# kaiwenShen/Do-You-Really-Need-to-Pay-2-20-Hedge-Fund-Strategy-Replication-via-Machine-Learning

Hardware: AMD Instinct MI355X
Metric: seq/sec/node MTSS-WGAN-GP train (24x32 windows) at 1/2/4/8 GPUs; W-dist parity (higher is better)
Workload: dtype fp32; 1 GPU; global_batch=262144, batch_per_gpu=262144, seq_len=24, features=32, parallelism=dp1

## Files before the change

do-you-really-need-to-pay-2-20-hedge-fund-strategy-replication-via-machine-learning_amd/csrc/lstm_f32.hip:

```cpp
#include "lstmf_dev.h"

#include <atomic>
#include <cstdlib>
#include <type_traits>
#include <stdexcept>

namespace hfrep {

namespace {

__device__ __forceinline__ rsrc_t ftile_rsrc(const float* base, int row0, int B, int Tn, int W) {
  row0 = __builtin_amdgcn_readfirstlane(row0);
  const int nr = base ? max(0, min(32, B - row0)) : 0;
  return make_rsrc(base + (nr ? (size_t)row0 * Tn * W : 0), nr * Tn * W * 4);
}

template <int K>
struct FGeo {
  static_assert(K >= 1 && K <= 112, "fp32 LSTM: K <= 112");
  static constexpr int KS = (K + 3) / 4;
  static constexpr int KQ = KS <= 12 ? 12 : 28;
  static constexpr int LR = KS <= 12 ? 56 : 120;
  static constexpr int NJ = (KS + 3) / 4;
};
// ... 965 lines not shown
            if (!tok) { cdn = 0.f; hd = 0.f; }
            cst[m][n] = cdn;
            cprev[m][n] = c;
            hv = hd;
            st4(f32x4{zd[0], zd[1], zd[2], zd[3]}, rt, tok ? tl + tb + ftape_slot(m, n) : kOOB);
            st1(cdn, rt, tok ? tcl + tb + ftape_slot(m, n) : kOOB, 0);
          }
          {
            const int u = ub + 4 * n, row = 16 * m + 4 * g + q;
            const uint32_t h1 = trunc_hi(hv);
            const float r1 = hv - __builtin_bit_cast(float, h1);
            const uint32_t m1 = trunc_hi(r1);
            const uint32_t l1 = __builtin_bit_cast(uint32_t, r1 - __builtin_bit_cast(float, m1));
            const bool pl = u < 96;
            lds_char* dp = pl ? hnext + (row * FS_HR + u) * 2 : trashc;
            *reinterpret_cast<__attribute__((address_space(3))) uint16_t*>(dp) = (uint16_t)(h1 >> 16);
            *reinterpret_cast<__attribute__((address_space(3))) uint16_t*>(dp + (pl ? FS_HPL : 0)) = (uint16_t)(m1 >> 16);
            *reinterpret_cast<__attribute__((address_space(3))) uint16_t*>(dp + (pl ? 2 * FS_HPL : 0)) = (uint16_t)(l1 >> 16);
            const bool tl4 = u >= 96 && u < FH;
            lds_char* tp = tl4 ? hnext + 3 * FS_HPL + (row * 4 + (u - 96)) * 4 : trashc;
            *reinterpret_cast<__attribute__((address_space(3))) float*>(tp) = hv;
          }
          st1(hv, rh, v1, 0);
        }
      }
      xp.to_lds(xb + ((t + 1) & 1) * 32 * GX::LR, trash);
      lds_barrier();
    }
  }
}

#ifndef HFREP_FWDS2_SKEW
#define HFREP_FWDS2_SKEW 0
#endif
constexpr int F2_TILES = 25;
__device__ __forceinline__ float f2_rnd(float v) {
  asm("" : "+v"(v));
  return v;
}
template <int KX>
constexpr size_t fwds2_smem() {
  return (size_t)(2 * 32 * FGeo<KX>::LR + 4) * 4 + 2 * FS_HB + (size_t)F2_TILES * FGeo<KX>::NJ * 64 * 16;
}

template <int ACT, int KX, bool TAPE, bool TAN, int NT, bool HI, bool FLIP>
__device__ __forceinline__ void fwds2_run(const float* __restrict__ x, const float* __restrict__ W,
                                          const float* __restrict__ bias, const float* __restrict__ U,
                                          const float* __restrict__ ptape, float* __restrict__ hs,
                                          float* __restrict__ tape, int B, int Tn, float* fsm, int v) {
  using GX = FGeo<KX>;
  float* xb = fsm;
  float* trash = xb + 2 * 32 * GX::LR;
  lds_char* hb = (lds_char*)(trash + 4);
  f32x4* wl = (f32x4*)(hb + 2 * FS_HB);
  const int tid = threadIdx.x, lane = tid & 63;
  const int q = lane & 3, g = lane >> 4, j4 = (lane & 15) >> 2;
  const int t0 = v ? 3 * v + 1 : 0;
  const int ub = 4 * t0 + j4;
  const int nrb = (B + 31) / 32;
  const int flip = (FLIP && v >= 4) ? 1 : 0;

  for (int i = tid; i < 2 * 32 * GX::LR; i += 512) xb[i] = 0.f;

  constexpr float GSC = ACT == ACT_TANH ? -2.f * kLog2e : ACT == ACT_SIGMOID ? -kLog2e : 1.f;
  const float sc = TAN ? 1.f : (q == 2 ? GSC : -kLog2e);
  bf16x8 up[3][NT][3];
  float ut[NT], bq[NT];
  int tsl[NT];
#pragma unroll
  for (int n = 0; n < NT; ++n) {
    const int cl = q * FH + ub + 4 * n;
    tsl[n] = ftape_lane((t0 + n) / FNT, 0) + (((t0 + n) % FNT) * FT_SLOT) * 4;
#pragma unroll
    for (int ks = 0; ks < 3; ++ks) {
      uint32_t hh[8], mm[8], ll[8];
#pragma unroll
      for (int j = 0; j < 8; ++j) {
        const int k = 32 * ks + 8 * g + j;
        const float u_ = f2_rnd(U[k * FG + cl] * sc);
        const uint32_t h = trunc_hi(u_);
        const float r1 = u_ - __builtin_bit_cast(float, h);
        const uint32_t m = trunc_hi(r1);
        const float r2 = r1 - __builtin_bit_cast(float, m);
        hh[j] = h; mm[j] = m; ll[j] = __builtin_bit_cast(uint32_t, r2);
      }
      uint4 ph, pm, pl;
      ph.x = __builtin_amdgcn_perm(hh[1], hh[0], 0x07060302u); ph.y = __builtin_amdgcn_perm(hh[3], hh[2], 0x07060302u);
      ph.z = __builtin_amdgcn_perm(hh[5], hh[4], 0x07060302u); ph.w = __builtin_amdgcn_perm(hh[7], hh[6], 0x07060302u);
      pm.x = __builtin_amdgcn_perm(mm[1], mm[0], 0x07060302u); pm.y = __builtin_amdgcn_perm(mm[3], mm[2], 0x07060302u);
      pm.z = __builtin_amdgcn_perm(mm[5], mm[4], 0x07060302u); pm.w = __builtin_amdgcn_perm(mm[7], mm[6], 0x07060302u);
      pl.x = __builtin_amdgcn_perm(ll[1], ll[0], 0x07060302u); pl.y = __builtin_amdgcn_perm(ll[3], ll[2], 0x07060302u);
      pl.z = __builtin_amdgcn_perm(ll[5], ll[4], 0x07060302u); pl.w = __builtin_amdgcn_perm(ll[7], ll[6], 0x07060302u);
      up[ks][n][0] = __builtin_bit_cast(bf16x8, ph);
      up[ks][n][1] = __builtin_bit_cast(bf16x8, pm);
      up[ks][n][2] = __builtin_bit_cast(bf16x8, pl);
#pragma unroll
      for (int p = 0; p < 3; ++p) asm volatile("" : "+v"(up[ks][n][p]));
    }
    ut[n] = U[(96 + g) * FG + cl] * sc;
#pragma unroll
    for (int j = 0; j < GX::NJ; ++j) {
      f32x4 wv;
#pragma unroll
      for (int s4 = 0; s4 < 4; ++s4) {
        const int k = 4 * (4 * j + s4) + g;
        const float w_ = W[min(k, KX - 1) * FG + cl];
        wv[s4] = k < KX ? w_ * sc : 0.f;
      }
      wl[((t0 + n) * GX::NJ + j) * 64 + lane] = wv;
    }
    const float bv = bias ? bias[cl] : 0.f;
    bq[n] = !TAN ? f2_rnd(bv * sc) : 0.f;
  }
  const bool glin = !TAN && ACT == ACT_LINEAR && q == 2;
  const float am = (ACT == ACT_TANH && q == 2) ? 2.f : 1.f, bm = (ACT == ACT_TANH && q == 2) ? -1.f : 0.f;
  const int ax = (lane & 15) * GX::LR + g * GX::KQ;
  const int ahp = ((lane & 15) * FS_HR + 8 * g) * 2, aht = 3 * FS_HPL + ((lane & 15) * 4 + g) * 4;
  const f32x4* wlw = wl + t0 * GX::NJ * 64 + lane;
  FXPart<KX> xp;
  const bool xld = v >= 4;

  for (int rb = blockIdx.x; rb < nrb; rb += gridDim.x) {
    const int row0 = rb * 32;
    const rsrc_t rx = ftile_rsrc(x, row0, B, Tn, KX);
    const rsrc_t rh = ftile_rsrc(hs, row0, B, Tn, FH);
    const rsrc_t rt = ftape_rsrc(TAPE ? tape : nullptr, rb, nrb, Tn);
    const rsrc_t rp = ftape_rsrc(TAN ? ptape : nullptr, rb, nrb, Tn);
    const int vp0 = ((4 * g + q) * Tn * FH + ub) * 4;
    float cprev[TAN ? 2 : 1][NT];
    if constexpr (TAN) {
#pragma unroll
      for (int i = 0; i < 2; ++i)
#pragma unroll
        for (int n = 0; n < NT; ++n) cprev[i][n] = 0.f;
    }
    float cst[2][NT];
#pragma unroll
    for (int i = 0; i < 2; ++i)
#pragma unroll
      for (int n = 0; n < NT; ++n) cst[i][n] = 0.f;
    xp.set(Tn, tid & 255);
    if (!xld) {
#pragma unroll
      for (int j = 0; j < FXPart<KX>::NJ; ++j) { xp.goff[j] = kOOB; xp.lpos[j] = -1; }
    }
    xp.load(rx, Tn, 0, true);
    for (int i = tid; i < FS_HB / 16; i += 512)
      reinterpret_cast<__attribute__((address_space(3))) u32x4_t*>(hb)[i] = u32x4_t{0, 0, 0, 0};
    xp.to_lds(xb, trash);
    __syncthreads();
    for (int t = 0; t < Tn; ++t) {
      const float* xcur = xb + (t & 1) * 32 * GX::LR;
      const lds_char* hcur = hb + (t & 1) * FS_HB;
      lds_char* hnext = hb + ((t + 1) & 1) * FS_HB;
      xp.load(rx, Tn, t + 1, t + 1 < Tn);
#pragma unroll
      for (int i = 0; i < 2; ++i) {
        const int m = i ^ flip;
        f32x4 pg[TAN ? NT : 1];
        float pc[TAN ? NT : 1];
        const int p1 = vp0 + (16 * m * Tn + t) * FH * 4;
        const int tb = t * FT_STEP * 4 + m * ftape_slot(1, 0);
        if constexpr (TAN) {
#pragma unroll
          for (int n = 0; n < NT; ++n) {
            pg[n] = ld4(rp, lane * 16 + (tb + tsl[n]));
            pc[n] = ld1(rp, (256 + lane) * 4 + (tb + tsl[n]), 0);
          }
        }
        f32x4 acc[NT];
#pragma unroll
        for (int n = 0; n < NT; ++n) acc[n] = f32x4{0.f, 0.f, 0.f, 0.f};
        if constexpr (HI) __builtin_amdgcn_s_setprio(1);
#pragma unroll
        for (int j = 0; j < GX::NJ; ++j) {
          const f32x4 a4 = *reinterpret_cast<const f32x4*>(xcur + ax + 16 * m * GX::LR + 4 * j);
          f32x4 w4[NT];
#pragma unroll
          for (int n = 0; n < NT; ++n) w4[n] = wlw[(n * GX::NJ + j) * 64];
#pragma unroll
          for (int s4 = 0; s4 < 4; ++s4) {
            const int ks = 4 * j + s4;
            if (ks >= GX::KS) break;
#pragma unroll
            for (int n = 0; n < NT; ++n) acc[n] = mma4(a4[s4], w4[n][s4], acc[n]);
          }
          __builtin_amdgcn_sched_barrier(0);
        }
#pragma unroll
        for (int ks = 0; ks < 3; ++ks) {
          const lds_char* ar = hcur + ahp + 16 * m * FS_HR * 2 + 64 * ks;
          const bf16x8 a[3] = {*reinterpret_cast<const __attribute__((address_space(3))) bf16x8*>(ar),
                               *reinterpret_cast<const __attribute__((address_space(3))) bf16x8*>(ar + FS_HPL),
                               *reinterpret_cast<const __attribute__((address_space(3))) bf16x8*>(ar + 2 * FS_HPL)};
#pragma unroll
          for (int n = 0; n < NT; ++n) acc[n] = mma_split6(a, up[ks][n], acc[n]);
          __builtin_amdgcn_sched_barrier(0);
        }
        {
          const float at = *reinterpret_cast<const __attribute__((address_space(3))) float*>(hcur + aht + 16 * m * 16);
#pragma unroll
          for (int n = 0; n < NT; ++n) acc[n] = mma4(at, ut[n], acc[n]);
        }
        if constexpr (HI) __builtin_amdgcn_s_setprio(0);
#pragma unroll
        for (int n = 0; n < NT; ++n) {
          const int v1 = p1 + 16 * n;
          const int tg = lane * 16 + (tb + tsl[n]), tc = (256 + lane) * 4 + (tb + tsl[n]);
          const bool fa = (t0 + n) % FNT < 4;
          const f32x4 zs = acc[n];
          float hv, hr;
          if constexpr (!TAN) {
            float y[4];
#pragma unroll
            for (int e4 = 0; e4 < 4; ++e4) {
              const float s_ = zs[e4] + bq[n];
              const float e = __builtin_fmaf(am, __builtin_amdgcn_rcpf(1.f + __builtin_amdgcn_exp2f(s_)), bm);
              y[e4] = glin ? s_ : e;
            }
            quad_transpose(y, q);
            const float cn = __builtin_fmaf(y[1], cst[i][n], y[0] * y[2]);
            float ca;
            if constexpr (ACT == ACT_TANH) ca = __builtin_fmaf(__builtin_amdgcn_rcpf(1.f + __builtin_amdgcn_exp2f(GSC * cn)), 2.f, -1.f);
            else if constexpr (ACT == ACT_SIGMOID) ca = __builtin_amdgcn_rcpf(1.f + __builtin_amdgcn_exp2f(GSC * cn));
            else ca = cn;
            hv = f2_rnd(y[3] * ca);
            const float hh = __builtin_bit_cast(float, trunc_hi(hv));
            hr = fa ? __builtin_fmaf(y[3], ca, -hh) : hv - hh;
            cst[i][n] = cn;
            if constexpr (TAPE) {
              st4(f32x4{y[0], y[1], y[2], y[3]}, rt, tg);
              st1(cn, rt, tc, 0);
            }
          } else {
            float zd[4] = {zs[0], zs[1], zs[2], zs[3]};
            quad_transpose(zd, q);
            const f32x4 y = pg[n];
            const float idot = y[0] * (1.f - y[0]) * zd[0], fdot = y[1] * (1.f - y[1]) * zd[1];
            const float dg = ACT == ACT_TANH ? __builtin_fmaf(-y[2], y[2], 1.f) : ACT == ACT_SIGMOID ? y[2] * (1.f - y[2]) : 1.f;
            const float gdot = dg * zd[2], odot = y[3] * (1.f - y[3]) * zd[3];
            const float c = pc[n];
            const float ca = act_f(ACT, c);
            const float dc = ACT == ACT_TANH ? __builtin_fmaf(-ca, ca, 1.f) : ACT == ACT_SIGMOID ? ca * (1.f - ca) : 1.f;
            const float yd = y[3] * dc;
            float cdn, hd;
            if (fa) {
              if constexpr (ACT == ACT_LINEAR) {
                cdn = f2_rnd(y[0] * gdot) + __builtin_fmaf(idot, y[2], __builtin_fmaf(fdot, cprev[i][n], y[1] * cst[i][n]));
              } else {
                cdn = __builtin_fmaf(y[0], gdot, f2_rnd(idot * y[2]) + (f2_rnd(y[1] * cst[i][n]) + f2_rnd(fdot * cprev[i][n])));
              }
              hd = f2_rnd(odot * ca) + f2_rnd(yd * cdn);
            } else {
              cdn = __builtin_fmaf(y[0], gdot, __builtin_fmaf(idot, y[2], __builtin_fmaf(y[1], cst[i][n], fdot * cprev[i][n])));
              hd = __builtin_fmaf(odot, ca, yd * cdn);
            }
            cst[i][n] = cdn;
            cprev[i][n] = c;
            hv = hd;
            hr = hv - __builtin_bit_cast(float, trunc_hi(hv));
            st4(f32x4{zd[0], zd[1], zd[2], zd[3]}, rt, tg);
            st1(cdn, rt, tc, 0);
          }
          {
            const int row = 16 * m + 4 * g + q;
            if (t0 + n < 24) {
              const uint32_t h1 = trunc_hi(hv);
              const uint32_t m1 = trunc_hi(hr);
              const uint32_t l1 = __builtin_bit_cast(uint32_t, hr - __builtin_bit_cast(float, m1));
              lds_char* dp = hnext + (row * FS_HR + ub + 4 * n) * 2;
              *reinterpret_cast<__attribute__((address_space(3))) uint16_t*>(dp) = (uint16_t)(h1 >> 16);
              *reinterpret_cast<__attribute__((address_space(3))) uint16_t*>(dp + FS_HPL) = (uint16_t)(m1 >> 16);
              *reinterpret_cast<__attribute__((address_space(3))) uint16_t*>(dp + 2 * FS_HPL) = (uint16_t)(l1 >> 16);
            } else {
              *reinterpret_cast<__attribute__((address_space(3))) float*>(hnext + 3 * FS_HPL + (row * 4 + j4) * 4) = hv;
            }
          }
          st1(hv, rh, v1, 0);
        }
      }
      xp.to_lds(xb + ((t + 1) & 1) * 32 * GX::LR, trash);
      lds_barrier();
    }
  }
}

template <int ACT, int KX, bool TAPE, bool TAN, int SKEW>
__global__ void __launch_bounds__(512, 1)
lstmf_fwds2_kernel(const float* __restrict__ x, const float* __restrict__ W, const float* __restrict__ bias,
                   const float* __restrict__ U, const float* __restrict__ ptape, float* __restrict__ hs,
                   float* __restrict__ tape, int B, int Tn) {
  static_assert(FGeo<KX>::KS <= 12, "split forward: K <= 48");
  extern __shared__ __attribute__((aligned(16))) float fsm[];
  constexpr bool PRIO = SKEW & 1, FLIP = SKEW & 2;
  const int v = __builtin_amdgcn_readfirstlane(threadIdx.x >> 6);
  if (v == 0) fwds2_run<ACT, KX, TAPE, TAN, 4, false, FLIP>(x, W, bias, U, ptape, hs, tape, B, Tn, fsm, v);
  else if (!PRIO || v < 4) fwds2_run<ACT, KX, TAPE, TAN, 3, false, FLIP>(x, W, bias, U, ptape, hs, tape, B, Tn, fsm, v);
  else fwds2_run<ACT, KX, TAPE, TAN, 3, true, FLIP>(x, W, bias, U, ptape, hs, tape, B, Tn, fsm, v);
}

constexpr int F2_NWR3 = 13, F2_NWR4 = 5;
constexpr int F2_G3 = (25 - F2_NWR3) / 4, F2_G4 = (25 - F2_NWR4) / 4;
static_assert(F2_NWR3 + 4 * F2_G3 == 25 && F2_NWR4 + 4 * F2_G4 == 25, "W^T k-steps in LDS come in fours");
__device__ __forceinline__ constexpr int f2_woff(int gt) { return gt < 4 ? F2_G4 * gt : F2_G3 * gt + (F2_G4 - F2_G3) * 4; }
constexpr size_t fwd2_smem() {
  return (size_t)(2 * 32 * (FGeo<100>::LR + FGeo<FH>::LR) + 4) * 4 + (size_t)(F2_G3 * 25 + (F2_G4 - F2_G3) * 4) * 1024;
}

template <int ACT, bool TAPE, bool TAN, int NT>
__device__ __forceinline__ void fwd2_run(const float* __restrict__ x, const float* __restrict__ W,
                                         const float* __restrict__ bias, const float* __restrict__ U,
                                         const float* __restrict__ ptape, float* __restrict__ hs,
                                         float* __restrict__ tape, int B, int Tn, float* fsm, int v) {
  constexpr int KX = 100;
  using GX = FGeo<KX>;
  using GH = FGeo<FH>;
  constexpr bool BIG = NT == 4;
  constexpr int NWR = BIG ? F2_NWR4 : F2_NWR3, NG = BIG ? F2_G4 : F2_G3;
  static_assert(GX::KS == 25 && GH::KS == 25 && (NT == 3 || NT == 4), "tile plan of the K = 100 layer");
  float* xb = fsm;
  float* hb = xb + 2 * 32 * GX::LR;
  float* trash = hb + 2 * 32 * GH::LR;
  f32x4* wl = (f32x4*)(trash + 4);
  const int tid = threadIdx.x, lane = tid & 63;
  const int q = lane & 3, g = lane >> 4, j4 = (lane & 15) >> 2;
  const int t0 = v ? 3 * v + 1 : 0;
  const int nrb = (B + 31) / 32;

  for (int i = tid; i < 2 * 32 * (GX::LR + GH::LR); i += 512) fsm[i] = 0.f;

  constexpr float GSC = ACT == ACT_TANH ? -2.f * kLog2e : ACT == ACT_SIGMOID ? -kLog2e : 1.f;
  const float sc = TAN ? 1.f : (q == 2 ? GSC : -kLog2e);
  float uf[GH::KS][NT], wf[NWR][NT], bq[NT];
  int tsl[NT];
#pragma unroll
  for (int n = 0; n < NT; ++n) {
    const int gt = t0 + n;
    const int cl = q * FH + 4 * gt + j4;
    tsl[n] = ftape_lane(gt / FNT, 0) + ((gt % FNT) * FT_SLOT) * 4;
#pragma unroll
    for (int ks = 0; ks < GH::KS; ++ks) {
      uf[ks][n] = U[(4 * ks + g) * FG + cl] * sc;
      asm volatile("" : "+v"(uf[ks][n]));
    }
#pragma unroll
    for (int ks = 0; ks < NWR; ++ks) {
      wf[ks][n] = W[(4 * ks + g) * FG + cl] * sc;
      asm volatile("" : "+v"(wf[ks][n]));
    }
#pragma unroll
    for (int gi = 0; gi < NG; ++gi) {
      f32x4 wv;
#pragma unroll
      for (int s4 = 0; s4 < 4; ++s4) wv[s4] = W[(4 * (NWR + 4 * gi + s4) + g) * FG + cl] * sc;
      wl[(f2_woff(gt) + gi) * 64 + lane] = wv;
    }
    const float bv = bias ? bias[cl] : 0.f;
    bq[n] = !TAN ? f2_rnd(bv * sc) : 0.f;
  }
  const bool glin = !TAN && ACT == ACT_LINEAR && q == 2;
  const float am = q == 2 ? 2.f : 1.f, bm = q == 2 ? -1.f : 0.f;
  const int ax = (lane & 15) * GX::LR + g * GX::KQ, ah = (lane & 15) * GH::LR + g * GH::KQ;
  const int hw = (4 * g + q) * GH::LR + j4 * GH::KQ + t0;
  const f32x4* wlw = wl + f2_woff(t0) * 64 + lane;
  FXPart<KX> xp;
  const bool xld = v >= 4;
  __syncthreads();

  for (int rb = blockIdx.x; rb < nrb; rb += gridDim.x) {
    const int row0 = rb * 32;
    const rsrc_t rx = ftile_rsrc(x, row0, B, Tn, KX);
    const rsrc_t rh = ftile_rsrc(hs, row0, B, Tn, FH);
    const rsrc_t rt = ftape_rsrc(TAPE ? tape : nullptr, rb, nrb, Tn);
    const rsrc_t rp = ftape_rsrc(TAN ? ptape : nullptr, rb, nrb, Tn);
    const int vp0 = ((4 * g + q) * Tn * FH + 4 * t0 + j4) * 4;
    float cprev[TAN ? 2 : 1][NT];
    if constexpr (TAN) {
#pragma unroll
      for (int m = 0; m < 2; ++m)
#pragma unroll
        for (int n = 0; n < NT; ++n) cprev[m][n] = 0.f;
    }
    float cst[2][NT];
#pragma unroll
    for (int m = 0; m < 2; ++m)
#pragma unroll
      for (int n = 0; n < NT; ++n) cst[m][n] = 0.f;
    if constexpr (!BIG) {
      xp.set(Tn, tid & 255);
      if (!xld) {
#pragma unroll
        for (int j = 0; j < FXPart<KX>::NJ; ++j) { xp.goff[j] = kOOB; xp.lpos[j] = -1; }
      }
      xp.load(rx, Tn, 0, true);
    }
    for (int i = tid; i < 32 * GH::LR; i += 512) hb[i] = 0.f;
    if constexpr (!BIG) xp.to_lds(xb, trash);
    __syncthreads();
    for (int t = 0; t < Tn; ++t) {
      const float* xcur = xb + (t & 1) * 32 * GX::LR;
      const float* hcur = hb + (t & 1) * 32 * GH::LR;
      float* hnext = hb + ((t + 1) & 1) * 32 * GH::LR;
      if constexpr (!BIG) xp.load(rx, Tn, t + 1, t + 1 < Tn);
#pragma unroll
      for (int m = 0; m < 2; ++m) {
        f32x4 pg[TAN ? NT : 1];
        float pc[TAN ? NT : 1];
        const int p1 = vp0 + (16 * m * Tn + t) * FH * 4;
        const int tb = t * FT_STEP * 4 + ftape_slot(m, 0);
        if constexpr (TAN) {
#pragma unroll
          for (int n = 0; n < NT; ++n) {
            pg[n] = ld4(rp, lane * 16 + (tb + tsl[n]));
            pc[n] = ld1(rp, (256 + lane) * 4 + (tb + tsl[n]), 0);
          }
        }
        f32x4 acc[NT];
#pragma unroll
        for (int n = 0; n < NT; ++n) acc[n] = f32x4{0.f, 0.f, 0.f, 0.f};
        f32x4 w4[NT];
#pragma unroll
        for (int j = 0; j < GX::NJ; ++j) {
          const f32x4 a4 = *reinterpret_cast<const f32x4*>(xcur + ax + 16 * m * GX::LR + 4 * j);
#pragma unroll
          for (int s = 0; s < 4; ++s) {
            const int ks = 4 * j + s;
            if (ks >= GX::KS) break;
            if (ks >= NWR && (ks - NWR) % 4 == 0) {
#pragma unroll
              for (int n = 0; n < NT; ++n) w4[n] = wlw[(n * NG + (ks - NWR) / 4) * 64];
            }
#pragma unroll
            for (int n = 0; n < NT; ++n) {
              const float bw = ks < NWR ? wf[ks < NWR ? ks : 0][n] : w4[n][(ks >= NWR ? ks - NWR : 0) & 3];
              acc[n] = mma4(a4[s], bw, acc[n]);
            }
          }
          __builtin_amdgcn_sched_barrier(0);
        }
#pragma unroll
        for (int j = 0; j < GH::NJ; ++j) {
          const f32x4 a4 = *reinterpret_cast<const f32x4*>(hcur + ah + 16 * m * GH::LR + 4 * j);
#pragma unroll
          for (int s = 0; s < 4; ++s) {
            const int ks = 4 * j + s;
            if (ks >= GH::KS) break;
#pragma unroll
            for (int n = 0; n < NT; ++n) acc[n] = mma4(a4[s], uf[ks][n], acc[n]);
          }
          __builtin_amdgcn_sched_barrier(0);
        }
#pragma unroll
        for (int n = 0; n < NT; ++n) {
          const int v1 = p1 + 16 * n;
          const int tg = lane * 16 + (tb + tsl[n]), tc = (256 + lane) * 4 + (tb + tsl[n]);
          const f32x4 zs = acc[n];
          float hv;
          if constexpr (!TAN) {
            float y[4];
#pragma unroll
            for (int e4 = 0; e4 < 4; ++e4) {
              const float s_ = zs[e4] + bq[n];
              const float r_ = __builtin_amdgcn_rcpf(1.f + __builtin_amdgcn_exp2f(s_));
              float e = r_;
              if constexpr (ACT == ACT_TANH) e = __builtin_fmaf(am, r_, bm);
              y[e4] = glin ? s_ : e;
            }
            quad_transpose(y, q);
            const float cn = __builtin_fmaf(y[1], cst[m][n], y[0] * y[2]);
            float ca;
            if constexpr (ACT == ACT_TANH) ca = __builtin_fmaf(__builtin_amdgcn_rcpf(1.f + __builtin_amdgcn_exp2f(GSC * cn)), 2.f, -1.f);
            else if constexpr (ACT == ACT_SIGMOID) ca = __builtin_amdgcn_rcpf(1.f + __builtin_amdgcn_exp2f(GSC * cn));
            else ca = cn;
            hv = y[3] * ca;
            cst[m][n] = cn;
            if constexpr (TAPE) {
              st4(f32x4{y[0], y[1], y[2], y[3]}, rt, tg);
              st1(cn, rt, tc, 0);
            }
          } else {
            float zd[4] = {zs[0], zs[1], zs[2], zs[3]};
            quad_transpose(zd, q);
            const f32x4 y = pg[n];
            const float idot = y[0] * (1.f - y[0]) * zd[0], fdot = y[1] * (1.f - y[1]) * zd[1];
            const float dg = ACT == ACT_TANH ? __builtin_fmaf(-y[2], y[2], 1.f) : ACT == ACT_SIGMOID ? y[2] * (1.f - y[2]) : 1.f;
            const float gdot = dg * zd[2], odot = y[3] * (1.f - y[3]) * zd[3];
            const float c = pc[n];
            const float ca = act_f(ACT, c);
            const float dc = ACT == ACT_TANH ? __builtin_fmaf(-ca, ca, 1.f) : ACT == ACT_SIGMOID ? ca * (1.f - ca) : 1.f;
            const float yd = y[3] * dc;
            const float fc = __builtin_fmaf(fdot, cprev[m][n], y[1] * cst[m][n]);
            float cdn = __builtin_fmaf(y[0], gdot, __builtin_fmaf(idot, y[2], fc));
            if (m == 0 && (t0 + n) % FNT == 4) {
              if constexpr (ACT == ACT_LINEAR) cdn = f2_rnd(y[0] * gdot) + (f2_rnd(idot * y[2]) + (f2_rnd(fdot * cprev[m][n]) + f2_rnd(y[1] * cst[m][n])));
              else cdn = __builtin_fmaf(y[0], gdot, f2_rnd(idot * y[2]) + fc);
            }
            hv = __builtin_fmaf(odot, ca, yd * cdn);
            cst[m][n] = cdn;
            cprev[m][n] = c;
            st4(f32x4{zd[0], zd[1], zd[2], zd[3]}, rt, tg);
            st1(cdn, rt, tc, 0);
          }
          hnext[hw + 16 * m * GH::LR + n] = hv;
          st1(hv, rh, v1, 0);
        }
      }
      if constexpr (!BIG) xp.to_lds(xb + ((t + 1) & 1) * 32 * GX::LR, trash);
      lds_barrier();
    }
  }
}

template <int ACT, int KX, bool TAPE, bool TAN>
__global__ void __launch_bounds__(512, 1)
lstmf_fwd2_kernel(const float* __restrict__ x, const float* __restrict__ W, const float* __restrict__ bias,
                  const float* __restrict__ U, const float* __restrict__ ptape, float* __restrict__ hs,
                  float* __restrict__ tape, int B, int Tn) {
  static_assert(KX == 100, "the eight-wave exact forward is the K = 100 layer's");
  extern __shared__ __attribute__((aligned(16))) float fsm[];
  const int v = __builtin_amdgcn_readfirstlane(threadIdx.x >> 6);
  if (v == 0) fwd2_run<ACT, TAPE, TAN, 4>(x, W, bias, U, ptape, hs, tape, B, Tn, fsm, v);
  else fwd2_run<ACT, TAPE, TAN, 3>(x, W, bias, U, ptape, hs, tape, B, Tn, fsm, v);
}

constexpr int BS_LZ = 432;
constexpr int BS_PL = 32 * BS_LZ * 2;

template <int ACT, bool HEAD = false, bool AHD = false>
__global__ void __launch_bounds__(256, 1)
lstmf_bwds_kernel(const float* __restrict__ dH, const float* __restrict__ tape, const float* __restrict__ U,
                  float* __restrict__ dZ, int B, int Tn, const float* __restrict__ hd, const float* __restrict__ hw,
                  float* __restrict__ aH) {
  extern __shared__ __attribute__((aligned(16))) float fsm[];
  float* zt = fsm;
  float* ht = zt + 32 * BZ_LR;
  float* trash = ht + 32 * BH_LR;
  lds_char* trashp = (lds_char*)(trash + 4 * BZ_KQ);
  lds_char* zp = (lds_char*)(trash + 4 * BZ_KQ + 4);
  const int tid = threadIdx.x, lane = tid & 63;
  const int w = __builtin_amdgcn_readfirstlane(tid >> 6);
  const int q = lane & 3, g = lane >> 4, j4 = (lane & 15) >> 2, c16 = lane & 15;
  const int nrb = (B + 31) / 32;
  bf16x8 up[2][DS_KS][3];
#pragma unroll
  for (int e = 0; e < 2; ++e) {
    const int col = 16 * (2 * w + e) + c16;
    const bool ok = col < FH;
#pragma unroll
    for (int ks = 0; ks < DS_KS; ++ks) {
      f32x4 v[2];
#pragma unroll
      for (int j = 0; j < 8; ++j) {
        const int k = min(32 * ks + 8 * g + j, FG - 1);
        const float x = U[(ok ? col : 0) * FG + (k & 3) * FH + (k >> 2)];
        v[j >> 2][j & 3] = (ok && 32 * ks + 8 * g + j < FG) ? x : 0.f;
      }
      uint32_t p0[3][2], p1[3][2];
      split3(v[0], p0);
      split3(v[1], p1);
#pragma unroll
      for (int p = 0; p < 3; ++p) {
        up[e][ks][p] = __builtin_bit_cast(bf16x8, make_uint4(p0[p][0], p0[p][1], p1[p][0], p1[p][1]));
        if (e == 1 || ks < 8) asm volatile("" : "+a"(up[e][ks][p]));
      }
    }
  }
  const int ub = FUW * w + j4;
  const int hr = (4 * g + q) * BH_LR + ub, zw = (4 * g + q) * BZ_LR + ub;
  const int zpw = ((4 * g + q) * BS_LZ + 4 * ub) * 2;
  const int ao = (c16 * BS_LZ + 8 * g) * 2;
  const RevStore st(tid, Tn);
  const int tl = ftape_lane(w, lane), tcl = ftape_cell(w, lane);
  for (int rb = blockIdx.x; rb < nrb; rb += gridDim.x) {
    const int row0 = rb * 32;
    const rsrc_t rdh = ftile_rsrc(dH, row0, B, Tn, FH), rt = ftape_rsrc(tape, rb, nrb, Tn);
    const rsrc_t rz = ftile_rsrc(dZ, row0, B, Tn, FG);
    const rsrc_t rah = ftile_rsrc(AHD ? aH : nullptr, row0, B, Tn, FH);
    const int nr = min(32, B - row0);
    int vp1[2];
#pragma unroll
    for (int m = 0; m < 2; ++m) vp1[m] = ((16 * m + 4 * g + q) * Tn * FH + ub) * 4;
    float hdv[2];
    head_rows<HEAD>(hdv, hd, true, row0, B, g, q);
    const rsrc_t rhw = head_rsrc<HEAD>(hw, Tn);
    const int hvo = ub * 4;
    float dc[2][FNT], tc[2][FNT];
    f32x4 tg[FNT];
    float tcp[FNT], tdh[FNT];
    const int T1 = Tn - 1;
#pragma unroll
    for (int n = 0; n < FNT; ++n) {
      const bool tok = unit_ok(w, n);
#pragma unroll
      for (int m = 0; m < 2; ++m) {
        dc[m][n] = 0.f;
        tc[m][n] = ld1(rt, tok ? tcl + T1 * FT_STEP * 4 + ftape_slot(m, n) : kOOB, 0);
      }
      bwdf_tape_load_u<HEAD>(tg[n], tcp[n], tdh[n], rt, rdh, tl, tcl, vp1[0], T1 * FT_STEP * 4 + ftape_slot(0, n),
                             max(T1 - 1, 0) * FT_STEP * 4 + ftape_slot(0, n), T1 * FH * 4 + 16 * n, tok, T1 > 0, hdv[0],
                             rhw, hvo);
    }
    for (int i = tid; i < 3 * BS_PL / 16; i += 256)
      reinterpret_cast<__attribute__((address_space(3))) u32x4_t*>(zp)[i] = u32x4_t{0, 0, 0, 0};
    for (int i = tid; i < 32 * BH_LR; i += 256) ht[i] = 0.f;
    __syncthreads();
    auto cell = [&](auto M_, int n, float hrec, int t) {
      constexpr int m = decltype(M_)::value;
      const bool tok = unit_ok(w, n);
      f32x4 z4;
      const float dht = bptt_cell<ACT>(z4, dc[m][n], tg[n], tc[m][n], tcp[n], tdh[n], hrec, tok,
                                       zt + zw + 16 * m * BZ_LR + 4 * n, trash);
      uint32_t p[3][2];
      split3(z4, p);
      planes_store(p, tok ? zp + zpw + 16 * m * BS_LZ * 2 + 32 * n : trashp, tok ? BS_PL : 0);
      tc[m][n] = tcp[n];
      if constexpr (m == 0) {
        bwdf_tape_load_u<HEAD>(tg[n], tcp[n], tdh[n], rt, rdh, tl, tcl, vp1[1], t * FT_STEP * 4 + ftape_slot(1, n),
                               max(t - 1, 0) * FT_STEP * 4 + ftape_slot(1, n), t * FH * 4 + 16 * n, tok, t > 0, hdv[1],
                               rhw, hvo);
      } else {
        const int tp = t > 0 ? t - 1 : 0;
        bwdf_tape_load_u<HEAD>(tg[n], tcp[n], tdh[n], rt, rdh, tl, tcl, vp1[0], tp * FT_STEP * 4 + ftape_slot(0, n),
                               max(tp - 1, 0) * FT_STEP * 4 + ftape_slot(0, n), tp * FH * 4 + 16 * n, tok && t > 0,
                               tp > 0, hdv[0], rhw, hvo);
      }
      if constexpr (AHD) st1(dht, rah, tok ? vp1[m] : kOOB, t * FH * 4 + 16 * n);
    };
    auto phase = [&](auto MA_, int t) {
      constexpr int MA = decltype(MA_)::value;
      if constexpr (MA == 1) {
        if (t < T1) st.half<1, false>(zt, rz, Tn, t + 1, nr);
      } else {
        st.half<0, false>(zt, rz, Tn, t, nr);
      }
      float hv[FNT];
#pragma unroll
      for (int n = 0; n < FNT; ++n) hv[n] = ht[hr + 16 * (1 - MA) * BH_LR + 4 * n];
      __builtin_amdgcn_sched_barrier(0);
      f32x4 acc[2] = {f32x4{0.f, 0.f, 0.f, 0.f}, f32x4{0.f, 0.f, 0.f, 0.f}};
      const lds_char* ar = zp + ao + 16 * MA * BS_LZ * 2;
      bf16x8 af[2][3];
#pragma unroll
      for (int p = 0; p < 3; ++p) af[0][p] = *reinterpret_cast<const __attribute__((address_space(3))) bf16x8*>(ar + p * BS_PL);
#pragma unroll
      for (int ks = 0; ks < DS_KS; ++ks) {
        if (ks + 1 < DS_KS) {
#pragma unroll
          for (int p = 0; p < 3; ++p)
            af[(ks + 1) & 1][p] = *reinterpret_cast<const __attribute__((address_space(3))) bf16x8*>(ar + p * BS_PL + 64 * (ks + 1));
        }
        const bf16x8(&a)[3] = af[ks & 1];
#pragma unroll
        for (int e = 0; e < 2; ++e) acc[e] = mma_split6(a, up[e][ks], acc[e]);
        if (ks < FNT) cell(std::integral_constant<int, 1 - MA>{}, ks, hv[ks], t);
      }
#pragma unroll
      for (int ks = 0; ks < DS_KS; ++ks) {
        __builtin_amdgcn_sched_group_barrier(0x100, 3, 0);
#pragma unroll
        for (int i = 0; i < 12; ++i) {
          __builtin_amdgcn_sched_group_barrier(0x008, 1, 0);
          __builtin_amdgcn_sched_group_barrier(0x002, 3, 0);
        }
      }
      __builtin_amdgcn_sched_barrier(0);
#pragma unroll
      for (int e = 0; e < 2; ++e) {
        const bool ok = 2 * w + e < 7;
        float* hd = ok ? ht + (16 * MA + 4 * g) * BH_LR + 16 * (2 * w + e) + c16 : trash;
        const int hs = ok ? BH_LR : 0;
#pragma unroll
        for (int i = 0; i < 4; ++i) hd[i * hs] = acc[e][i];
      }
      lds_barrier();
    };
    for (int t = T1; t >= 0; --t) {
      phase(I1{}, t);
      phase(I0{}, t);
    }
    st.half<1, false>(zt, rz, Tn, 0, nr);
    __syncthreads();
  }
}

namespace {
template <int KX>
constexpr size_t fwdf_smem() {
  return (size_t)(2 * 32 * FGeo<KX>::LR + 2 * 32 * FGeo<FH>::LR + f_nwl<KX>() * 4 * FNT * 64 + 4) * 4;
}
static_assert(fwdf_smem<100>() <= F_LDS_MAX, "fp32 forward LDS");

template <int KX>
constexpr size_t fwds_smem() {
  return (size_t)(2 * 32 * FGeo<KX>::LR) * 4 + 2 * FS_HB + 16;
}
static_assert(fwds2_smem<32>() <= F_LDS_MAX, "two-wave split forward LDS");
static_assert(fwd2_smem() <= F_LDS_MAX, "eight-wave exact forward LDS");
static std::atomic<int>& fwdf_impl() {
  static std::atomic<int> v{fp32_exact() ? 1 : 3};
  return v;
}
static int fwdf_version() { return fwdf_impl().load(std::memory_order_relaxed); }
static std::atomic<int>& fwdf100_impl() {
  static std::atomic<int> v{2};
  return v;
}
template <int ACT, int KX, bool TAPE, bool TAN>
void fwd2_launch(const float* x, const float* W, const float* b, const float* U, const float* pt, float* hs, float* tp,
                 int B, int Tn, hipStream_t s) {
  const int nrb = (B + 31) / 32, cus = device_cu_count();
  auto k = lstmf_fwd2_kernel<ACT, KX, TAPE, TAN>;
  allow_lds(reinterpret_cast<const void*>(k));
  hipLaunchKernelGGL(k, dim3(nrb < cus ? nrb : cus), dim3(512), fwd2_smem(), s, x, W, b, U, pt, hs, tp, B, Tn);
}
template <int ACT, int KX, bool TAPE, bool TAN, int SKEW>
void fwds2_launch(const float* x, const float* W, const float* b, const float* U, const float* pt, float* hs, float* tp,
                  int B, int Tn, hipStream_t s) {
  const int nrb = (B + 31) / 32, cus = device_cu_count();
  auto k = lstmf_fwds2_kernel<ACT, KX, TAPE, TAN, SKEW>;
  allow_lds(reinterpret_cast<const void*>(k));
  hipLaunchKernelGGL(k, dim3(nrb < cus ? nrb : cus), dim3(512), fwds2_smem<KX>(), s, x, W, b, U, pt, hs, tp, B, Tn);
}
template <int ACT, int KX, bool TAPE, bool TAN>
void fwdf_launch(const float* x, const float* W, const float* b, const float* U, const float* pt, float* hs, float* tp,
                 int B, int Tn, hipStream_t s) {
  const int nrb = (B + 31) / 32, cus = device_cu_count();
  if constexpr (KX == 100) {
    if (fwdf100_impl().load(std::memory_order_relaxed) == 2)
      return fwd2_launch<ACT, KX, TAPE, TAN>(x, W, b, U, pt, hs, tp, B, Tn, s);
  }
  if constexpr (KX == 32) {
    const int ver = fwdf_version();
    if (ver == 3) return fwds2_launch<ACT, KX, TAPE, TAN, HFREP_FWDS2_SKEW>(x, W, b, U, pt, hs, tp, B, Tn, s);
#ifdef HFREP_FWDS2_AB
    if constexpr (ACT == ACT_TANH) {
      if (ver == 30) return fwds2_launch<ACT, KX, TAPE, TAN, 0>(x, W, b, U, pt, hs, tp, B, Tn, s);
      if (ver == 31) return fwds2_launch<ACT, KX, TAPE, TAN, 1>(x, W, b, U, pt, hs, tp, B, Tn, s);
      if (ver == 32) return fwds2_launch<ACT, KX, TAPE, TAN, 2>(x, W, b, U, pt, hs, tp, B, Tn, s);
      if (ver == 33) return fwds2_launch<ACT, KX, TAPE, TAN, 3>(x, W, b, U, pt, hs, tp, B, Tn, s);
    }
#endif
  }
  if constexpr (FGeo<KX>::KS <= 8 || (FGeo<KX>::KS <= 12 && !TAN)) {
    if (fwdf_version() >= 2) {
      auto k = lstmf_fwds_kernel<ACT, KX, TAPE, TAN>;
      allow_lds(reinterpret_cast<const void*>(k));
      hipLaunchKernelGGL(k, dim3(nrb < cus ? nrb : cus), dim3(256), fwds_smem<KX>(), s, x, W, b, U, pt, hs, tp, B, Tn);
      return;
    }
  }
  auto k = lstmf_fwd_kernel<ACT, KX, TAPE, TAN>;
  allow_lds(reinterpret_cast<const void*>(k));
  hipLaunchKernelGGL(k, dim3(nrb < cus ? nrb : cus), dim3(256), fwdf_smem<KX>(), s, x, W, b, U, pt, hs, tp, B, Tn);
}
template <int KX, bool TAPE, bool TAN>
void fwdf_act(int act, const float* x, const float* W, const float* b, const float* U, const float* pt, float* hs,
              float* tp, int B, int Tn, hipStream_t s) {
  switch (act) {
    case ACT_LINEAR: fwdf_launch<ACT_LINEAR, KX, TAPE, TAN>(x, W, b, U, pt, hs, tp, B, Tn, s); break;
    case ACT_SIGMOID: fwdf_launch<ACT_SIGMOID, KX, TAPE, TAN>(x, W, b, U, pt, hs, tp, B, Tn, s); break;
    default: fwdf_launch<ACT_TANH, KX, TAPE, TAN>(x, W, b, U, pt, hs, tp, B, Tn, s); break;
  }
}
template <bool TAPE, bool TAN>
bool fwdf_k(int K, int act, const float* x, const float* W, const float* b, const float* U, const float* pt, float* hs,
            float* tp, int B, int Tn, hipStream_t s) {
  switch (K) {
    case 32: fwdf_act<32, TAPE, TAN>(act, x, W, b, U, pt, hs, tp, B, Tn, s); return true;
    case 35: fwdf_act<35, TAPE, TAN>(act, x, W, b, U, pt, hs, tp, B, Tn, s); return true;
    case 36: fwdf_act<36, TAPE, TAN>(act, x, W, b, U, pt, hs, tp, B, Tn, s); return true;
    case 100: fwdf_act<100, TAPE, TAN>(act, x, W, b, U, pt, hs, tp, B, Tn, s); return true;
    default: return false;
  }
}
}

int set_lstmf_fwd_impl(int v) { return fwdf_impl().exchange(v); }
int set_lstmf_fwd100_impl(int v) { return fwdf100_impl().exchange(v); }

bool lstmf_supported(int H, int K, int act) {
  return H == FH && (K == 32 || K == 35 || K == 36 || K == 100) && (act == ACT_LINEAR || act == ACT_SIGMOID || act == ACT_TANH);
}

bool launch_lstmf_fwd(const float* x, const float* W, const float* b, const float* U, float* hs, float* tape, int B,
                      int Tn, int K, int H, int act, hipStream_t s) {
  if (!lstmf_supported(H, K, act) || B <= 0 || Tn <= 0) return false;
  if (tape) return fwdf_k<true, false>(K, act, x, W, b, U, nullptr, hs, tape, B, Tn, s);
  return fwdf_k<false, false>(K, act, x, W, b, U, nullptr, hs, nullptr, B, Tn, s);
}

bool launch_lstmf_tfwd(const float* xd, const float* W, const float* U, const float* tape, float* hds, float* ttape,
                       int B, int Tn, int K, int H, int act, hipStream_t s) {
  if (!lstmf_supported(H, K, act) || B <= 0 || Tn <= 0) return false;
  return fwdf_k<true, true>(K, act, xd, W, nullptr, U, tape, hds, ttape, B, Tn, s);
}

static std::atomic<int>& bwdf_impl() {
  static std::atomic<int> v{fp32_exact() ? 2 : 3};
  return v;
}
template <int ACT>
void bwdf_launch(const float* dH, const float* tape, const float* U, float* dZ, int B, int Tn, hipStream_t s,
                 const float* hd, const float* hw, float* aH) {
  const int ver = bwdf_impl().load(std::memory_order_relaxed);
  const int nrb = (B + 31) / 32, cus = device_cu_count();
  const size_t sm = (size_t)(32 * BZ_LR + 32 * BH_LR + 4 * BZ_KQ) * 4;
  if (ver != 2) {
    auto go = [&](auto k) {
      allow_lds(reinterpret_cast<const void*>(k));
      hipLaunchKernelGGL(k, dim3(nrb < cus ? nrb : cus), dim3(256), sm + 16 + 3 * BS_PL, s, dH, tape, U, dZ, B, Tn, hd,
                         hw, aH);
    };
    if (aH) {
      if (hd) go(lstmf_bwds_kernel<ACT, true, true>);
      else go(lstmf_bwds_kernel<ACT, false, true>);
    } else {
      if (hd) go(lstmf_bwds_kernel<ACT, true>);
      else go(lstmf_bwds_kernel<ACT, false>);
    }
    return;
  }
  if (aH) throw std::runtime_error("lstmf_bwd: the exact-fp32 BPTT does not store the h adjoints (lstmf_ahd_supported)");
  if (hd) throw std::runtime_error("lstmf_bwd: the exact-fp32 BPTT takes a materialised dH (lstmf_head_supported)");
  auto k = lstmf_bwdp_kernel<ACT>;
  allow_lds(reinterpret_cast<const void*>(k));
// ... 69 lines not shown
```

Measured before the change: 1.597 million seq/s.

## Split the extra K=100 forward gate tile across two waves by row half

In the eight-wave K=100 forward kernel, wave 0 used to own four gate tiles (0-3) while the other waves owned three. Now waves 0 and 1 each own three tiles plus a shared 25th tile, with each wave computing that tile for only one of the two 16-row halves. The remaining waves shift their tile offsets, the LDS weight layout is reordered to match, and the x-prefetch assignment moves to waves 2,3,6,7. The aim is to balance the per-wave MMA load on the serial timestep critical path. In exchange the code adds a per-half lambda with a variable tile count and a more complex weight-offset map.

```diff
diff --git a/do-you-really-need-to-pay-2-20-hedge-fund-strategy-replication-via-machine-learning_amd/csrc/lstm_f32.hip b/do-you-really-need-to-pay-2-20-hedge-fund-strategy-replication-via-machine-learning_amd/csrc/lstm_f32.hip
--- a/do-you-really-need-to-pay-2-20-hedge-fund-strategy-replication-via-machine-learning_amd/csrc/lstm_f32.hip
+++ b/do-you-really-need-to-pay-2-20-hedge-fund-strategy-replication-via-machine-learning_amd/csrc/lstm_f32.hip
@@ -1291,12 +1291,16 @@
 constexpr int F2_NWR3 = 13, F2_NWR4 = 5;
 constexpr int F2_G3 = (25 - F2_NWR3) / 4, F2_G4 = (25 - F2_NWR4) / 4;
 static_assert(F2_NWR3 + 4 * F2_G3 == 25 && F2_NWR4 + 4 * F2_G4 == 25, "W^T k-steps in LDS come in fours");
-__device__ __forceinline__ constexpr int f2_woff(int gt) { return gt < 4 ? F2_G4 * gt : F2_G3 * gt + (F2_G4 - F2_G3) * 4; }
+template <int ROLE>
+__device__ __forceinline__ constexpr int f2_rel(int n) { return n < 3 ? n : 24 - 3 * (ROLE - 1); }
+__device__ __forceinline__ constexpr int f2_woff(int gt) {
+  return gt < 6 ? F2_G4 * gt : gt == 24 ? F2_G4 * 6 : F2_G4 * 7 + F2_G3 * (gt - 6);
+}
 constexpr size_t fwd2_smem() {
-  return (size_t)(2 * 32 * (FGeo<100>::LR + FGeo<FH>::LR) + 4) * 4 + (size_t)(F2_G3 * 25 + (F2_G4 - F2_G3) * 4) * 1024;
-}
-
-template <int ACT, bool TAPE, bool TAN, int NT>
+  return (size_t)(2 * 32 * (FGeo<100>::LR + FGeo<FH>::LR) + 4) * 4 + (size_t)(F2_G4 * 7 + F2_G3 * 18) * 1024;
+}
+
+template <int ACT, bool TAPE, bool TAN, int ROLE>
 __device__ __forceinline__ void fwd2_run(const float* __restrict__ x, const float* __restrict__ W,
                                          const float* __restrict__ bias, const float* __restrict__ U,
                                          const float* __restrict__ ptape, float* __restrict__ hs,
@@ -1304,16 +1308,17 @@
   constexpr int KX = 100;
   using GX = FGeo<KX>;
   using GH = FGeo<FH>;
-  constexpr bool BIG = NT == 4;
+  constexpr bool BIG = ROLE != 0;
+  constexpr int NT = BIG ? 4 : 3;
   constexpr int NWR = BIG ? F2_NWR4 : F2_NWR3, NG = BIG ? F2_G4 : F2_G3;
-  static_assert(GX::KS == 25 && GH::KS == 25 && (NT == 3 || NT == 4), "tile plan of the K = 100 layer");
+  static_assert(GX::KS == 25 && GH::KS == 25 && ROLE >= 0 && ROLE <= 2, "tile plan of the K = 100 layer");
   float* xb = fsm;
   float* hb = xb + 2 * 32 * GX::LR;
   float* trash = hb + 2 * 32 * GH::LR;
   f32x4* wl = (f32x4*)(trash + 4);
   const int tid = threadIdx.x, lane = tid & 63;
   const int q = lane & 3, g = lane >> 4, j4 = (lane & 15) >> 2;
-  const int t0 = v ? 3 * v + 1 : 0;
+  const int t0 = BIG ? 3 * (ROLE - 1) : 3 * v;
   const int nrb = (B + 31) / 32;
 
   for (int i = tid; i < 2 * 32 * (GX::LR + GH::LR); i += 512) fsm[i] = 0.f;
@@ -1324,7 +1329,7 @@
   int tsl[NT];
 #pragma unroll
   for (int n = 0; n < NT; ++n) {
-    const int gt = t0 + n;
+    const int gt = t0 + f2_rel<ROLE>(n);
     const int cl = q * FH + 4 * gt + j4;
     tsl[n] = ftape_lane(gt / FNT, 0) + ((gt % FNT) * FT_SLOT) * 4;
 #pragma unroll
@@ -1342,7 +1347,7 @@
       f32x4 wv;
 #pragma unroll
       for (int s4 = 0; s4 < 4; ++s4) wv[s4] = W[(4 * (NWR + 4 * gi + s4) + g) * FG + cl] * sc;
-      wl[(f2_woff(gt) + gi) * 64 + lane] = wv;
+      if (n < 3 || ROLE == 1) wl[(f2_woff(gt) + gi) * 64 + lane] = wv;
     }
     const float bv = bias ? bias[cl] : 0.f;
     bq[n] = !TAN ? f2_rnd(bv * sc) : 0.f;
@@ -1352,8 +1357,11 @@
   const int ax = (lane & 15) * GX::LR + g * GX::KQ, ah = (lane & 15) * GH::LR + g * GH::KQ;
   const int hw = (4 * g + q) * GH::LR + j4 * GH::KQ + t0;
   const f32x4* wlw = wl + f2_woff(t0) * 64 + lane;
+  constexpr int WR24 = BIG ? f2_woff(24) - f2_woff(3 * (ROLE - 1)) : 0;
+  auto wrel = [](int n) constexpr { return n < 3 ? n * NG : WR24; };
   FXPart<KX> xp;
-  const bool xld = v >= 4;
+  const bool xld = (v & 2) != 0;
+  const int xtid = (((v >> 2) << 1) | (v & 1)) * 64 + lane;
   __syncthreads();
 
   for (int rb = blockIdx.x; rb < nrb; rb += gridDim.x) {
@@ -1376,7 +1384,7 @@
 #pragma unroll
       for (int n = 0; n < NT; ++n) cst[m][n] = 0.f;
     if constexpr (!BIG) {
-      xp.set(Tn, tid & 255);
+      xp.set(Tn, xtid);
       if (!xld) {
 #pragma unroll
         for (int j = 0; j < FXPart<KX>::NJ; ++j) { xp.goff[j] = kOOB; xp.lpos[j] = -1; }
@@ -1391,23 +1399,24 @@
       const float* hcur = hb + (t & 1) * 32 * GH::LR;
       float* hnext = hb + ((t + 1) & 1) * 32 * GH::LR;
       if constexpr (!BIG) xp.load(rx, Tn, t + 1, t + 1 < Tn);
-#pragma unroll
-      for (int m = 0; m < 2; ++m) {
-        f32x4 pg[TAN ? NT : 1];
-        float pc[TAN ? NT : 1];
+      auto half = [&](auto M_) {
+        constexpr int m = decltype(M_)::value;
+        constexpr int NH = (BIG && m == ROLE - 1) ? 4 : 3;
+        f32x4 pg[TAN ? NH : 1];
+        float pc[TAN ? NH : 1];
         const int p1 = vp0 + (16 * m * Tn + t) * FH * 4;
         const int tb = t * FT_STEP * 4 + ftape_slot(m, 0);
         if constexpr (TAN) {
 #pragma unroll
-          for (int n = 0; n < NT; ++n) {
+          for (int n = 0; n < NH; ++n) {
             pg[n] = ld4(rp, lane * 16 + (tb + tsl[n]));
             pc[n] = ld1(rp, (256 + lane) * 4 + (tb + tsl[n]), 0);
           }
         }
-        f32x4 acc[NT];
-#pragma unroll
-        for (int n = 0; n < NT; ++n) acc[n] = f32x4{0.f, 0.f, 0.f, 0.f};
-        f32x4 w4[NT];
+        f32x4 acc[NH];
+#pragma unroll
+        for (int n = 0; n < NH; ++n) acc[n] = f32x4{0.f, 0.f, 0.f, 0.f};
+        f32x4 w4[NH];
 #pragma unroll
         for (int j = 0; j < GX::NJ; ++j) {
           const f32x4 a4 = *reinterpret_cast<const f32x4*>(xcur + ax + 16 * m * GX::LR + 4 * j);
@@ -1417,10 +1426,10 @@
             if (ks >= GX::KS) break;
             if (ks >= NWR && (ks - NWR) % 4 == 0) {
 #pragma unroll
-              for (int n = 0; n < NT; ++n) w4[n] = wlw[(n * NG + (ks - NWR) / 4) * 64];
+              for (int n = 0; n < NH; ++n) w4[n] = wlw[(wrel(n) + (ks - NWR) / 4) * 64];
             }
 #pragma unroll
-            for (int n = 0; n < NT; ++n) {
+            for (int n = 0; n < NH; ++n) {
               const float bw = ks < NWR ? wf[ks < NWR ? ks : 0][n] : w4[n][(ks >= NWR ? ks - NWR : 0) & 3];
               acc[n] = mma4(a4[s], bw, acc[n]);
             }
@@ -1435,13 +1444,13 @@
             const int ks = 4 * j + s;
             if (ks >= GH::KS) break;
 #pragma unroll
-            for (int n = 0; n < NT; ++n) acc[n] = mma4(a4[s], uf[ks][n], acc[n]);
+            for (int n = 0; n < NH; ++n) acc[n] = mma4(a4[s], uf[ks][n], acc[n]);
           }
           __builtin_amdgcn_sched_barrier(0);
         }
 #pragma unroll
-        for (int n = 0; n < NT; ++n) {
-          const int v1 = p1 + 16 * n;
+        for (int n = 0; n < NH; ++n) {
+          const int v1 = p1 + 16 * f2_rel<ROLE>(n);
           const int tg = lane * 16 + (tb + tsl[n]), tc = (256 + lane) * 4 + (tb + tsl[n]);
           const f32x4 zs = acc[n];
           float hv;
@@ -1480,7 +1489,7 @@
             const float yd = y[3] * dc;
             const float fc = __builtin_fmaf(fdot, cprev[m][n], y[1] * cst[m][n]);
             float cdn = __builtin_fmaf(y[0], gdot, __builtin_fmaf(idot, y[2], fc));
-            if (m == 0 && (t0 + n) % FNT == 4) {
+            if (m == 0 && (t0 + f2_rel<ROLE>(n)) % FNT == 4) {
               if constexpr (ACT == ACT_LINEAR) cdn = f2_rnd(y[0] * gdot) + (f2_rnd(idot * y[2]) + (f2_rnd(fdot * cprev[m][n]) + f2_rnd(y[1] * cst[m][n])));
               else cdn = __builtin_fmaf(y[0], gdot, f2_rnd(idot * y[2]) + fc);
             }
@@ -1490,10 +1499,12 @@
             st4(f32x4{zd[0], zd[1], zd[2], zd[3]}, rt, tg);
             st1(cdn, rt, tc, 0);
           }
-          hnext[hw + 16 * m * GH::LR + n] = hv;
+          hnext[hw + 16 * m * GH::LR + f2_rel<ROLE>(n)] = hv;
           st1(hv, rh, v1, 0);
         }
-      }
+      };
+      half(I0{});
+      half(I1{});
       if constexpr (!BIG) xp.to_lds(xb + ((t + 1) & 1) * 32 * GX::LR, trash);
       lds_barrier();
     }
@@ -1508,8 +1519,9 @@
   static_assert(KX == 100, "the eight-wave exact forward is the K = 100 layer's");
   extern __shared__ __attribute__((aligned(16))) float fsm[];
   const int v = __builtin_amdgcn_readfirstlane(threadIdx.x >> 6);
-  if (v == 0) fwd2_run<ACT, TAPE, TAN, 4>(x, W, bias, U, ptape, hs, tape, B, Tn, fsm, v);
-  else fwd2_run<ACT, TAPE, TAN, 3>(x, W, bias, U, ptape, hs, tape, B, Tn, fsm, v);
+  if (v == 0) fwd2_run<ACT, TAPE, TAN, 1>(x, W, bias, U, ptape, hs, tape, B, Tn, fsm, v);
+  else if (v == 1) fwd2_run<ACT, TAPE, TAN, 2>(x, W, bias, U, ptape, hs, tape, B, Tn, fsm, v);
+  else fwd2_run<ACT, TAPE, TAN, 0>(x, W, bias, U, ptape, hs, tape, B, Tn, fsm, v);
 }
 
 constexpr int BS_LZ = 432;
```

After: 1.620 million seq/s (median of 6 runs). +1.4%, better.
